# Dylan-H-Wang/skin-sm3

Measured on AMD Instinct MI355X. Metric: SM3 pretrain images/sec (paired 224x224), higher is better.
Workload: dtype bf16

## Files before the change

### include/sm3_hip.h

```cpp
#ifndef SM3_HIP_H
#define SM3_HIP_H

#include <stdint.h>

#ifdef __cplusplus
extern "C" {
#endif

#define SM3_F32 0
#define SM3_BF16 1
#define SM3_F16 2

#define SM3_EINVAL (-1)
#define SM3_EALIGN (-2)
#define SM3_EDTYPE (-3)

#define SM3_MAX_TAPS 9

int sm3_abi_version(void);

typedef struct sm3_conv_desc {
    int32_t dtype;
    int32_t N, Hi, Wi, Ci;
    int32_t Ho, Wo, Co;
// ... 54 lines not shown
int sm3_conv_wgrad_slabs(const sm3_conv_desc* d, const void* x, const void* dy, float* slabs, int slab_capacity, int views,
                         int* slabs_used, void* stream);
int sm3_slab_reduce(const float* slabs, int nslabs, int64_t n, float* out, int accumulate, void* stream);
int sm3_conv_wgrad_det(const sm3_conv_desc* d, const void* x, const void* dy, float* dw, float* slabs, int slab_capacity,
                       void* stream);

#define SM3_BN_REDUCE_GROUPS 64
int sm3_bn_reduce_groups(int rows);
int sm3_bn_stats_reduce(const float* partials, int rows, int C, double* sums, double* workspace, int views,
                        void* stream);
int sm3_bn_finalize(const double* sums, int groups , int views,
                    double count , int C, const float* gamma, const float* beta,
                    float eps, float momentum, float* running_mean, float* running_var,
                    int64_t* num_batches_tracked , float* scale, float* shift, float* save_mean,
                    float* save_invstd , void* stream);
int sm3_bn_eval_scale_shift(const float* gamma, const float* beta, const float* running_mean,
                            const float* running_var, float eps, int C, float* scale, float* shift,
                            void* stream);
int sm3_bn_act(int dtype, const void* x, const float* scale, const float* shift, const void* residual,
               int relu, int out_f32, void* y, uint8_t* relu_mask, int64_t rows, int C, int views, void* stream);
int sm3_bn_act_colsum_rows(int64_t rows, int C, int dtype);
int sm3_bn_act_colsum(int dtype, const void* x, const float* scale, const float* shift, const void* residual, int relu,
                      void* y, uint8_t* relu_mask, float* colsum_partials, int64_t rows, int C, int views, void* stream);
int sm3_subsample_colsum_rows(int64_t rows, int C, int dtype);
int sm3_subsample_colsum(int dtype, const void* x, void* y, float* colsum_partials, int N, int H, int W, int C, int stride,
                         int views, void* stream);
int sm3_bn_add_bn_act(int dtype, const void* x, const float* scale, const float* shift, const void* x2,
                      const float* scale2, const float* shift2, int relu, void* y, uint8_t* relu_mask,
                      int64_t rows, int C, int views, void* stream);
int sm3_bn_bwd_partial_rows(int64_t rows, int C);
int sm3_bn_bwd_reduce(int dtype, const void* dy, const void* y, const uint8_t* relu_mask, const void* x,
                      const float* mean, const float* invstd, void* dz, int64_t rows, int C,
                      float* partials , int views, void* stream);
int sm3_bn_bwd_apply(int dtype, const void* dz, const void* x, const float* mean, const float* invstd,
                     const float* gamma, const double* global_sums, double count,
                     const double* local_sums, float* dgamma, float* dbeta, void* dx, int64_t rows,
                     int C, int views, void* stream);

typedef struct sm3_bn_apply_side {
    const void* x;
    const float* mean;
    const float* invstd;
    const float* gamma;
    const double* global_sums;
    const double* local_sums;
    float* dgamma;
// ... 246 lines not shown
```

### skin-sm3_amd/csrc/bn.hip

```cpp
#include "common.h"
#include <cstdlib>

namespace {

struct RowWalk {
    int tbx, tby;
    int gx, gy;
};
static RowWalk make_walk(int64_t rows, int cvecs, int max_gy, int views = 1) {
    RowWalk w;
    if (cvecs >= 256) {
        w.tbx = 256;
    } else {
        w.tbx = cvecs;
    }
    w.tby = 256 / w.tbx;
    if (w.tby < 1) w.tby = 1;
    w.gx = (cvecs + w.tbx - 1) / w.tbx;
    int64_t gy = (rows + (int64_t)w.tby * 8 - 1) / ((int64_t)w.tby * 8);
    static const int grid_cap = getenv("SM3_BN_GRID_CAP") ? atoi(getenv("SM3_BN_GRID_CAP")) : 768;
    const int64_t cap = grid_cap / (w.gx * views) > 0 ? grid_cap / (w.gx * views) : 1;
    if (gy > cap) gy = cap;
    if (gy > max_gy) gy = max_gy;
    if (gy < 1) gy = 1;
// ... 269 lines not shown
#pragma unroll
                for (int e = 0; e < E; ++e) cs[e] += q[e];
            }
        }
        for (; r < rows; r += rstep) {
            const uint4 xu = ldg16<false>(x + src_row(r) * C + (int64_t)cv * E);
            if (y) stg16<true>(y + (r_lo + r) * C + (int64_t)cv * E, xu);
            float q[E];
            unpack16<T>(xu, q);
#pragma unroll
            for (int e = 0; e < E; ++e) cs[e] += q[e];
        }
    }
    if constexpr (E <= 8) {
#pragma unroll
        for (int e = 0; e < E; ++e) scol[threadIdx.x * E + e] = cs[e];
    }
    __syncthreads();
    if (active && ty == 0) {
        for (int j = 1; j < tby; ++j)
#pragma unroll
            for (int e = 0; e < E; ++e) cs[e] += scol[(j * tbx + tx) * E + e];
        float* o = colsum + ((int64_t)blockIdx.z * gridDim.y + blockIdx.y) * C + (int64_t)cv * E;
#pragma unroll
        for (int e = 0; e < E; ++e) o[e] = cs[e];
    }
}

template <typename T, int U, bool NT>
__global__ __launch_bounds__(256) void bn_bwd_reduce_kernel(const T* __restrict__ dy, const T* __restrict__ y,
                                                            const uint8_t* __restrict__ mask,
                                                            const T* __restrict__ x, const float* __restrict__ mean,
                                                            const float* __restrict__ invstd, T* __restrict__ dz,
                                                            int64_t rows, int C, float* __restrict__ partials,
                                                            int tbx, int tby) {
    constexpr int E = ElemTraits<T>::kPer16B;
    __shared__ float sred[256 * 2 * 8];
    const int tx = threadIdx.x % tbx, ty = threadIdx.x / tbx;
    const int cv = blockIdx.x * tbx + tx;
    const bool active = (cv * E < C) && (ty < tby);
    {
        const int64_t vo = (int64_t)blockIdx.z * rows * C;
        dy += vo;
        if (x) {
            x += vo;
            mean += (int64_t)blockIdx.z * C;
// ... 392 lines not shown
    if (!SM3_DTYPE_OK(dtype)) return SM3_EDTYPE;
    const int E = dtype == SM3_F32 ? 4 : 8;
    if (C % E) return SM3_EALIGN;
    const int Hs = (H - 1) / stride + 1, Ws = (W - 1) / stride + 1;
    const int64_t rows = (int64_t)(N / views) * Hs * Ws;
    if ((int64_t)N * Hs * Ws > 0x7fffffffL) return SM3_EINVAL;
    const RowWalk w = make_walk(rows, C / E, 8192, views < 2 ? 2 : views);
    dim3 grid(w.gx, w.gy, views), block(256);
    const FastDiv dhw = make_fastdiv((uint32_t)(Hs * Ws)), dw = make_fastdiv((uint32_t)Ws);
    hipStream_t st = (hipStream_t)stream;
    if (dtype == SM3_F32)
        hipLaunchKernelGGL((subsample_colsum_kernel<float, 4>), grid, block, 0, st, (const float*)x, (float*)y, colsum_partials, rows,
                           C, Hs, Ws, H, W, stride, dhw, dw, w.tbx, w.tby);
    else if (dtype == SM3_BF16)
        hipLaunchKernelGGL((subsample_colsum_kernel<bf16_t, 4>), grid, block, 0, st, (const bf16_t*)x, (bf16_t*)y, colsum_partials,
                           rows, C, Hs, Ws, H, W, stride, dhw, dw, w.tbx, w.tby);
    else
        hipLaunchKernelGGL((subsample_colsum_kernel<f16_t, 4>), grid, block, 0, st, (const f16_t*)x, (f16_t*)y, colsum_partials,
                           rows, C, Hs, Ws, H, W, stride, dhw, dw, w.tbx, w.tby);
    SM3_CHECK_LAUNCH();
    return 0;
}

extern "C" int sm3_bn_add_bn_act(int dtype, const void* x, const float* scale, const float* shift, const void* x2,
                                 const float* scale2, const float* shift2, int relu, void* y, uint8_t* relu_mask,
                                 int64_t rows, int C, int views, void* stream) {
    if (!x2 || !scale2 || !shift2) return SM3_EINVAL;
    return bn_act_impl(dtype, x, scale, shift, x2, scale2, shift2, relu, 0, y, relu_mask, rows, C, views, stream);
}

static int bwd_gy(int64_t rows) {
    int64_t gy = (rows + 63) / 64;
    if (gy > 1024) gy = 1024;
    if (gy < 1) gy = 1;
    return (int)gy;
}

extern "C" int sm3_bn_bwd_partial_rows(int64_t rows, int C) {
    (void)C;
    return rows > 0 ? bwd_gy(rows) : SM3_EINVAL;
}

extern "C" int sm3_bn_bwd_reduce(int dtype, const void* dy, const void* y, const uint8_t* relu_mask, const void* x,
                                 const float* mean, const float* invstd, void* dz, int64_t rows, int C,
                                 float* partials, int views, void* stream) {
    if (!dy || (x && (!mean || !invstd)) || !partials || rows <= 0 || C <= 0 || views < 1) return SM3_EINVAL;
// ... 74 lines not shown
```

### skin-sm3_amd/sm3hip/_lib.py

```python
import ctypes as C
import os

_HERE = os.path.dirname(os.path.abspath(__file__))
LIB_PATH = os.environ.get("SM3_LIBRARY") or os.path.join(_HERE, "libsm3hip.so")

SM3_F32, SM3_BF16, SM3_F16 = 0, 1, 2
MAX_TAPS = 9


class ConvDesc(C.Structure):
    _fields_ = [
        ("dtype", C.c_int32),
        ("N", C.c_int32), ("Hi", C.c_int32), ("Wi", C.c_int32), ("Ci", C.c_int32),
        ("Ho", C.c_int32), ("Wo", C.c_int32), ("Co", C.c_int32),
        ("sy", C.c_int32), ("sx", C.c_int32),
        ("ntaps", C.c_int32),
        ("dy", C.c_int32 * MAX_TAPS), ("dx", C.c_int32 * MAX_TAPS), ("wtap", C.c_int32 * MAX_TAPS),
        ("w_row_stride", C.c_int32),
        ("Hout", C.c_int32), ("Wout", C.c_int32),
        ("osy", C.c_int32), ("osx", C.c_int32), ("ooy", C.c_int32), ("oox", C.c_int32),
    ]


class BnBwdFuse(C.Structure):
# ... 27 lines not shown
    "sm3_conv_gather_gemm": [_DESC, _P, _P, _P, _P, _P, _P],
    "sm3_conv_dgrad_bnfuse": [_DESC, _P, _P, _P, _P, _P, _P],
    "sm3_conv_dgrad_seg_bnfuse": [_DESC, _P, _P, _P, _P, _P, _P, _P],
    "sm3_conv_gather_gemm_seg": [_DESC, _P, _P, _P, _P, _P, _P],
    "sm3_conv_seg_act": [_DESC, _P, _P, _P, _I, _P, _P, _P],
    "sm3_linbn_fold": [_P, _I, _I, _I, _P, _P],
    "sm3_p2p_mailbox_bytes": [],
    "sm3_p2p_max_elems": [],
    "sm3_p2p_max_world": [],
    "sm3_p2p_layout": [_I, _I, _I, _P, _P, _P, _P],
    "sm3_p2p_alloc": [_P, _P, _P],
    "sm3_p2p_open": [_P, _P],
    "sm3_p2p_close": [_P],
    "sm3_p2p_free": [_P],
    "sm3_p2p_allreduce_f64": [_P, _I, _P, _I, _I, C.c_uint64, _P, _D, _P],
    "sm3_linbn_scale_banks": [_I, _P, _I, _P, _P, _P, _P, _I, _P, _P, _P, _P, _I, _I, _P],
    "sm3_subsample_colsum_rows": [_L, _I, _I],
    "sm3_subsample_colsum": [_I, _P, _P, _P, _I, _I, _I, _I, _I, _I, _P],
    "sm3_conv_wgrad_cat": [_DESC, _P, _P, _P, _P, _I, _P, _I, _L, _L, _P],
    "sm3_bn_act_colsum_rows": [_L, _I, _I],
    "sm3_conv_wgrad_slabs": [_DESC, _P, _P, _P, _I, _I, _P, _P],
    "sm3_linbn_moments": [_P, _I, _L, _P, _P, _I, _P, _I, _I, _P],
    "sm3_bn_act_colsum": [_I, _P, _P, _P, _P, _I, _P, _P, _P, _L, _I, _I, _P],
    "sm3_conv_bn_act_fused": [_DESC, _P, _P, _P, _P, _P, _I, _P, _P, _I, _P],
    "sm3_linbn_fwd_stats": [_I, _P, _P, _P, _P, _P, _P, _I, _I, _I, _P],
    "sm3_linbn_stats": [_I, _P, _P, _P, _P, _P, _P, _I, _P, _P, _P, _D, _P, _I, _I, _I, _P],
    "sm3_linbn_coef": [_P, _D, _P, _P, _P, _P, _I, _I, _P],
    "sm3_linbn_banks": [_I, _P, _P, _P, _P, _P, _I, _I, _I, _P],
    "sm3_linbn_post": [_I, _P, _P, _P, _P, _P, _P, _P, _P, _P, _I, _I, _I, _P],
    "sm3_linbn_banks_post": [_I, _P, _P, _P, _P, _P, _P, _P, _P, _P, _P, _I, _I, _I, _P],
    "sm3_conv_bn_act_eval": [_DESC, _P, _P, _P, _P, _P, _I, _P, _P],
    "sm3_conv_bn_eval": [_DESC, _P, _P, _P, _P, _P, _P, _F, _P, _I, _P, _P],
    "sm3_conv_wgrad": [_DESC, _P, _P, _P, _P],
    "sm3_conv_wgrad_det": [_DESC, _P, _P, _P, _P, _I, _P],
    "sm3_slab_reduce": [_P, _I, _L, _P, _I, _P],
    "sm3_bn_stats_reduce": [_P, _I, _I, _P, _P, _I, _P],
    "sm3_bn_reduce_groups": [_I],
    "sm3_bn_finalize": [_P, _I, _I, _D, _I, _P, _P, _F, _F, _P, _P, _P, _P, _P, _P, _P, _P],
    "sm3_bn_eval_scale_shift": [_P, _P, _P, _P, _F, _I, _P, _P, _P],
    "sm3_bn_act": [_I, _P, _P, _P, _P, _I, _I, _P, _P, _L, _I, _I, _P],
    "sm3_bn_add_bn_act": [_I, _P, _P, _P, _P, _P, _P, _I, _P, _P, _L, _I, _I, _P],
    "sm3_bn_bwd_apply2": [_I, _P, _D, _P, _P, _L, _I, _I, _P],
    "sm3_bn_relu_maxpool_fwd": [_I, _P, _P, _P, _P, _P, _I, _I, _I, _I, _I, _P],
    "sm3_maxpool_bn_bwd_partial_rows": [_I, _I, _I, _I],
    "sm3_maxpool_bn_bwd": [_I, _P, _P, _P, _P, _P, _P, _P, _P, _P, _I, _I, _I, _I, _I, _P],
    "sm3_bn_bwd_partial_rows": [_L, _I],
# ... 131 lines not shown
```

### skin-sm3_amd/sm3hip/engine.py

```python
import os
from collections import OrderedDict
from contextlib import contextmanager

import torch

from . import ops
from ._lib import SM3_BF16, SM3_F16
from .plan import (TWO_PASS, BlockRec, EncoderCtx, ParamStore, ProjectorPlan, Rec, block_form, enc_mod_out_dim, enc_plan,
                   stage_of)
from .plan import EncoderPlan

BN_EPS = 1e-5
BN_MOMENTUM = 0.1


_LANE_POOL = {}


def lane_stream_pool(device, n):
    idx = device.index if device.index is not None else torch.cuda.current_device()
    pool = _LANE_POOL.setdefault(idx, [])
    if len(pool) >= n:
        return pool[:n]
    if os.environ.get("SM3_STREAM_CALIBRATE", "1") == "0" or not hasattr(torch.cuda, "_sleep"):
        pool.extend(torch.cuda.Stream(device=device) for _ in range(n - len(pool)))
        return pool[:n]
    import time
    main = torch.cuda.current_stream(device)
    cyc = 1_000_000

    def spin(a, b):
        torch.cuda.synchronize(device)
        t0 = time.perf_counter()
        with torch.cuda.stream(a):
            torch.cuda._sleep(cyc)
# ... 62 lines not shown
        self._allocated = False
        self._lane = "main"
        self._V = 1
        self._data_only = False
        self._no_stat_update = False
        self.weights_dirty = True
        self._wprep_cache, self._wprep_key, self._hash_tracks_banks = {}, None, False
        self._lane_prep = {}
        self._lin_descs = {}
        self.last_feats = None
        self._faith_saved_bytes = {}
        self.pair_views = os.environ.get("SM3_PAIR_VIEWS", "1") != "0"
        self.two_streams = True
        self._streams, self._streams_dev = None, None
        self.linbn = self.dtype in (SM3_BF16, SM3_F16) and os.environ.get("SM3_LINBN", "1") != "0"
        self.linbn_fwd = os.environ.get("SM3_LINBN_FWD", "1") != "0"
        self.linbn_ds = os.environ.get("SM3_LINBN_DS", "1") != "0"
        self.linbn_join = os.environ.get("SM3_LINBN_JOIN", "1") != "0"
        self.linbn_merge = os.environ.get("SM3_LINBN_MERGE", "1") != "0"
        self.lane_cross = os.environ.get("SM3_LANE_CROSS", "1") != "0"
        if self.cross is not None and self.cross[0] is self.cross[1]:
            self.lane_cross = False
        self.det_wgrad = os.environ.get("SM3_WGRAD_DET", "1") != "0"
        self.stem16 = self.dtype in (SM3_BF16, SM3_F16) and os.environ.get("SM3_STEM16", "1") != "0"

    def _all_conv_units(self):
        seen = set()
        plans = [p for pair in self.branches.values() for p in pair if p is not None]
        plans += list(self.cross or ())
        if self.meta is not None:
            plans.append(self.meta)
        for plan in plans:
            for cu in plan.conv_units():
                if id(cu) not in seen:
                    seen.add(id(cu))
                    yield cu

    def prepare(self, device):
        if self.store is None or self.store.flat_p.device != device:
            self.store = ParamStore(self.module, device)
            self._allocated = False
        else:
            self.store.rebind_if_needed()
        if not self._allocated:
            for cu in self._all_conv_units():
                cu.alloc(self.dtype, device)
# ... 131 lines not shown
            rm, rv = self.buffers[bu.name + ".running_mean"], self.buffers[bu.name + ".running_var"]
            nbt = self.buffers[bu.name + ".num_batches_tracked"]
        ops.bn_finalize(sums, count, bu.C, gamma, beta, BN_EPS, BN_MOMENTUM, rm, rv, nbt, scale, shift, mean, invstd,
                        groups=groups, views=V)

    @contextmanager
    def _views(self, V):
        self._V = V
        try:
            yield
        finally:
            self._V = 1

    @contextmanager
    def _params_backward(self, params):
        prev = self._data_only
        self._data_only = prev or not params
        try:
            yield
        finally:
            self._data_only = prev

    def conv_bn(self, cu, bu, x, N, H, W, relu, residual=None, train=True, save=False, out_f32=False, y_out=None,
                apply=True, scale_shift=None, res_affine=None, pending=None, colsum=None):
        dev = x.t.device if isinstance(x, ops.StemImage) else x.device
        direct = cu.stem
        if direct:
            d = None
            Ho, Wo = (H - 1) // 2 + 1, (W - 1) // 2 + 1
        else:
            d = cu.fwd_desc(self.dtype, N, H, W)
            Ho, Wo = d.Ho, d.Wo
        rows = N * Ho * Wo
        C = cu.Co
        V = self._V if train else 1
        rows_v = rows // V
        xo = torch.empty(rows, C, dtype=self.tdt, device=dev)
        scale, shift = scale_shift if scale_shift is not None else (self._work("scale", 2 * 2048),
                                                                    self._work("shift", 2 * 2048))
        mean = invstd = None

        def convolve(partials):
            if direct:
                (ops.stem_conv_fwd16 if isinstance(x, ops.StemImage) else ops.stem_conv_fwd)(self.dtype, x, cu.w_fwd, xo, partials)
            elif cu.groups > 1:
                ops.gconv_fwd(self.dtype, x, cu.w_fwd, xo, partials, N, H, W, C, cu.groups, cu.stride)
            else:
# ... 45 lines not shown
                if y_out is None:
                    y_out = xo
                ops.conv_bn_eval(d, x, cu.w_fwd, gamma, beta, rm, rv, BN_EPS, residual, relu, y_out)
                return y_out, Ho, Wo, None
            convolve(None)
            ops.bn_eval_scale_shift(gamma, beta, rm, rv, BN_EPS, C, scale, shift)
            if save:
                mean, invstd = rm.clone(), torch.rsqrt(rv + BN_EPS)
        mask = None
        if not apply:
            y_out = None
        else:
            if y_out is None:
                y_out = torch.empty(rows, C, dtype=torch.float32 if out_f32 else self.tdt, device=dev)
            if save and relu:
                mask = torch.empty(rows * C // (16 // ops._sz(self.dtype)), dtype=torch.uint8, device=dev)
            cs = None
            if res_affine is not None:
                ops.bn_add_bn_act(self.dtype, xo, scale, shift, residual, res_affine[0], res_affine[1], relu, y_out,
                                  rows_v, C, mask=mask, views=V)
            else:
                if colsum is not None and save and train and not out_f32:
                    cs = colsum
                ops.bn_act(self.dtype, xo, scale, shift, residual, relu, y_out, rows_v, C, out_f32=out_f32, mask=mask,
                           views=V, colsum=cs)
        r = None
        if save:
            r = Rec(cu, bu, N, H, W, Ho, Wo, x_in=x, xo=xo, mean=mean, invstd=invstd, y=y_out, relu=relu, mask=mask, V=V,
                    frozen_stats=not train, colsum=cs if apply else None)
        return (y_out if apply else xo), Ho, Wo, r

    def _phase1(self, r, dy, fused_rows):
        if fused_rows is not None:
            return fused_rows, self._ws[(self._lane, "fz_partials")]
        C, V = r.cu.Co, r.V
        rows = r.N * r.Ho * r.Wo // V
        prow = ops.bn_bwd_partial_rows(rows, C)
        bpart = self._work("partials", V * prow * 2 * C)
        ops.bn_bwd_reduce(self.dtype, dy, None, r.xo, r.mean, r.invstd, dy if r.relu else None, rows, C, bpart,
                          mask=r.mask if r.relu else None, views=V)
        return prow, bpart

    def bn_backward(self, r, dy, keep_dz, fused_rows=None):
        C = r.cu.Co
        V = r.V
        rows = r.xo.shape[0] // V
        prow, bpart = self._phase1(r, dy, fused_rows)
        lsums, gsums, count = self._bn_backward_sums(r, bpart, prow)
# ... 32 lines not shown
        ops.bn_stats_reduce(dpart, prow_d, C, lsums[n:], views=V)
        gsums, count = lsums, rows
        if r3.frozen_stats:
            gsums = self._work("zsums2", 2 * 2 * 2 * 2048, torch.float64)
            gsums.zero_()
        elif self.stat_sync is not None:
            gsums = self._work("gsums2", 2 * 2 * 2 * 2048, torch.float64)
            gsums[: 2 * n].copy_(lsums[: 2 * n])
            self.stat_sync(gsums[: 2 * n])
            count = rows * self.world_size
        dx3 = torch.empty_like(r3.xo)

        def side(r, g, l, dx):
            dgamma, dbeta = self._bn_affine(r.bu, grad=True)
            return dict(x=r.xo, mean=r.mean, invstd=r.invstd, gamma=self._bn_affine(r.bu)[0], gsums=g, lsums=l,
                        dgamma=dgamma, dbeta=dbeta, dx=dx)
        ops.bn_bwd_apply2(self.dtype, dy, count, side(r3, gsums[:n], lsums[:n], dx3),
                          side(rd, gsums[n: 2 * n], lsums[n: 2 * n], dy), rows, C, views=V)
        return dx3, dy

    def _slab_buf(self, n, V):
        cap = max(1, min(ops.SLAB_CAP, (1 << 24) // n))
        return self._work("linbn_slabs", V * cap * n), cap

    def _lin_conv_desc(self, dtype, N, H, W, Ci, Co):
        cache = self._lin_descs
        key = ("conv", dtype, N, H, W, Ci, Co)
        if key not in cache:
            cache[key] = ops.fwd_desc(dtype, N, H, W, Ci, Co, 1, 1, 0)
        return cache[key]

    def conv3_bn3_fused(self, cu, bu, r2, y2, idn, N, H, W):
        dev = y2.device
        C, p, V = cu.Co, cu.Ci, self._V
        d = cu.fwd_desc(self.dtype, N, H, W)
        rows = N * d.Ho * d.Wo
        rows_v = rows // V
        if V > 1 and rows_v % 128:
            raise ValueError("two views in one batch need a multiple of 128 rows per view")
        Tm = torch.empty(V * C * p, dtype=torch.float32, device=dev)
        groups = p // 32
        ws = self._work("linbn_fws", V * groups * 2 * C, torch.float64)
        ops.linbn_fwd_stats(self.dtype, r2.gram, cu.w_dgrad, cu.w_fwd, r2.colsum, Tm, ws, C, p, V)
        count = rows_v
        if self.stat_sync is not None:
            gs = self._work("linbn_fold", 2 * V * 2 * C, torch.float64)
# ... 41 lines not shown
        for bu, wsl, groups, tag in units:
            scale, shift = self._work("scale" + tag, 2 * 2048), self._work("shift" + tag, 2 * 2048)
            mean = torch.empty(V * C, dtype=torch.float32, device=dev)
            invstd = torch.empty(V * C, dtype=torch.float32, device=dev)
            self._bn_finalize(bu, wsl, count, scale, shift, mean, invstd, groups, V)
            out.append((scale, shift, mean, invstd))
        (sc3, sh3, mean3, inv3), (scd, shd, meand, invd) = out
        w3s = self._work("linbn_w3s", V * C * p, self.tdt)
        wds = self._work("linbn_wds", V * C * Cin, self.tdt)
        bias = self._work("linbn_fbias", V * C)
        ops.linbn_scale_banks(self.dtype, c3.w_fwd, sc3, sh3, w3s, cd.w_fwd, scd, shd, wds, bias, C, V)
        y3 = torch.empty(M, C, dtype=self.tdt, device=dev)
        mask = torch.empty(M * C // (16 // ops._sz(self.dtype)), dtype=torch.uint8, device=dev)
        ops.conv_seg_act(self._lin_conv_desc(self.dtype, N, h2, w2, p, C), y2, w3s, in_s, wds, bias, y3, mask, True,
                         views=V, w_view_stride=C * p, w1_view_stride=C * Cin)
        rd = Rec(cd, bd, N, h, w, h2, w2, x_in=cur, mean=meand, invstd=invd, V=V, linbn=True, in_s=in_s, gram=Gd, colsum=sd,
                 Tm=Tmd)
        r3 = Rec(c3, b3, N, h2, w2, h2, w2, x_in=y2, mean=mean3, invstd=inv3, y=y3, relu=True, mask=mask, V=V, linbn=True,
                 Tm=Tm3)
        return y3, h2, w2, rd, r3

    def _strided_input_moments(self, cd, x, N, h, w, hs, ws, V, keep):
        Cin, M = cd.Ci, N * hs * ws
        crow = ops.subsample_colsum_rows(self.dtype, M // V, Cin)
        csd = self._work("linbn_cs", V * crow * Cin)
        in_s = x if cd.stride == 1 else torch.empty(M, Cin, dtype=self.tdt, device=x.device)
        ops.subsample_colsum(self.dtype, x, None if cd.stride == 1 else in_s, csd, N, h, w, Cin, cd.stride, V)
        slabs, cap = self._slab_buf(Cin * Cin, V)
        ns = ops.conv_wgrad_slabs(self._lin_conv_desc(self.dtype, N, hs, ws, Cin, Cin), in_s, in_s, slabs, views=V, cap=cap)
        if keep:
            Gd = torch.empty(V * Cin * Cin, dtype=torch.float32, device=x.device)
            sd = torch.empty(V * Cin, dtype=torch.float64, device=x.device)
        else:
            Gd = self._work("linbn_Gd", V * Cin * Cin)
            sd = self._work("linbn_sd", V * Cin, torch.float64)
        ops.linbn_moments(slabs, ns, Cin * Cin, Gd, views=V, colsum=csd, colsum_rows=crow, s_out=sd, p=Cin)
        return in_s, Gd, sd

    def _lin_unit_products(self, tag, cu, N, Hs, Ws, y_in, dz, V):
        C, p = cu.Co, cu.Ci
        slabs, cap = self._slab_buf(C * p, V)
        ns = ops.conv_wgrad_slabs(self._lin_conv_desc(self.dtype, N, Hs, Ws, p, C), y_in, dz, slabs, views=V, cap=cap)
        P = self._work("linbn_P" + tag, V * C * p)
        ops.linbn_moments(slabs, ns, C * p, P, views=V)
        return P

    def _lin_unit_finish(self, tag, cu, P, G, Tm, s, coef, V):
        C, p = cu.Co, cu.Ci
        wa = self._work("linbn_wa" + tag, V * p * C, self.tdt)
        cconst = self._work("linbn_const" + tag, V * p)
        Hn = self._work("linbn_H" + tag, V * p * p, self.tdt)
        if self.linbn_merge:
# ... 206 lines not shown

    def _identity_branch(self, blk, cur, N, h, w, train, save):
        if "cd" not in blk:
            return cur, None, None, None
        if not (train or save):
            return self.conv_bn(blk["cd"], blk["bd"], cur, N, h, w, False, None, train)[0], None, None, None
        ra = (self._work("scale_d", 2 * 2048), self._work("shift_d", 2 * 2048))
        pend = [] if (train and self.stat_sync is not None) else None
        idn, _, _, rd = self.conv_bn(blk["cd"], blk["bd"], cur, N, h, w, False, None, train, save, apply=False,
                                     scale_shift=ra, pending=pend)
        return idn, ra, pend, rd

    def _basic_forward(self, blk, form, cur, N, h, w, train, save):
        y1, h1, w1, r1 = self.conv_bn(blk["c1"], blk["b1"], cur, N, h, w, True, None, train, save)
        idn, ra, pend, rd = self._identity_branch(blk, cur, N, h, w, train, save)
        y2, h2, w2, r2 = self.conv_bn(blk["c2"], blk["b2"], y1, N, h1, w1, True, idn, train, save, res_affine=ra,
                                      pending=pend)
        return y2, h2, w2, (BlockRec(form, r1, r2, rd=rd) if save else None)

    def _bottleneck_forward(self, blk, form, cur, N, h, w, train, save):
        V = self._V
        y1, h1, w1, r1 = self.conv_bn(blk["c1"], blk["b1"], cur, N, h, w, True, None, train, save)
        pp = blk["c3"].Ci
        cs = crow = None
        if form.lin:
            d2 = blk["c2"].fwd_desc(self.dtype, N, h1, w1)
            crow = ops.bn_act_colsum_rows(self.dtype, N * d2.Ho * d2.Wo // V, pp)
            cs = self._work("linbn_cs", V * crow * pp)
        y2, h2, w2, r2 = self.conv_bn(blk["c2"], blk["b2"], y1, N, h1, w1, True, None, train, save, colsum=cs)
        if form.lin:
            slabs, cap = self._slab_buf(pp * pp, V)
            ns = ops.conv_wgrad_slabs(self._lin_conv_desc(self.dtype, N, h2, w2, pp, pp), y2, y2, slabs, views=V, cap=cap)
            r2.gram = torch.empty(V * pp * pp, dtype=torch.float32, device=y2.device)
            r2.colsum = torch.empty(V * pp, dtype=torch.float64, device=y2.device)
            ops.linbn_moments(slabs, ns, pp * pp, r2.gram, views=V, colsum=cs, colsum_rows=crow, s_out=r2.colsum, p=pp)
        if form.join_fused:
            y3, h3, w3, rd, r3 = self.join_fused(blk, r2, y2, cur, N, h, w, h2, w2)
        else:
            idn, ra, pend, rd = self._identity_branch(blk, cur, N, h, w, train, save)
            if form.conv3_fused:
                y3, h3, w3, r3 = self.conv3_bn3_fused(blk["c3"], blk["b3"], r2, y2, idn, N, h2, w2)
            else:
                y3, h3, w3, r3 = self.conv_bn(blk["c3"], blk["b3"], y2, N, h2, w2, True, idn, train, save, res_affine=ra,
                                              pending=pend)
                if form.lin:
                    r3.linbn = True
        return y3, h3, w3, (BlockRec(form, r1, r2, r3, rd) if save else None)

    def encoder_backward(self, ctx, dfeat, last_view=True, taps=None, dx_out=None, params=True, stop_at=None):
        with self._params_backward(params):
            return self._encoder_backward(ctx, dfeat, last_view, taps, dx_out, stop_at)

    def _stop_block(self, ctx, stop_at):
        names = [stage_of(b) for b in ctx.plan.blocks]
        if stop_at not in names or names[-1] == stop_at:
# ... 326 lines not shown
```

### skin-sm3_amd/sm3hip/ops.py

```python
import ctypes as C

import torch

from . import _lib
from ._lib import ConvDesc, SM3_BF16, SM3_F16, SM3_F32, check

TORCH_DTYPE = {SM3_F32: torch.float32, SM3_BF16: torch.bfloat16, SM3_F16: torch.float16}
K_CHUNK = {SM3_F32: 32, SM3_BF16: 64, SM3_F16: 64}


_PROFILER = None


def set_profiler(p):
    global _PROFILER
    _PROFILER = p


class _prof:
    __slots__ = ("tag", "flops", "nbytes", "start")

    def __init__(self, tag, flops=0.0, nbytes=0.0):
        self.tag, self.flops, self.nbytes, self.start = tag, flops, nbytes, None

# ... 836 lines not shown
    if x.numel() != n or y.numel() != n or (residual is not None and residual.numel() != n):
        raise ValueError("bn_act: size mismatch")
    if scale.numel() < views * Cn or shift.numel() < views * Cn:
        raise ValueError("bn_act: scale/shift too small")
    _chk(mask, torch.uint8, "mask")
    if mask is not None and mask.numel() != n // (16 // _sz(dtype)):
        raise ValueError("bn_act: mask size mismatch")
    tag = "bn_act"
    if _PROFILER is not None and getattr(_PROFILER, "detail", False):
        tag += f"|rows{views * rows}_C{Cn}_res{int(residual is not None)}"
    _chk(colsum, torch.float32, "colsum")
    if colsum is not None and (out_f32 or colsum.numel() < views * bn_act_colsum_rows(dtype, rows, Cn) * Cn):
        raise ValueError("bn_act: colsum needs the storage dtype and [views][colsum_rows][C] floats")
    with _prof(tag, 0.0, _sz(dtype) * n * (2 if residual is None else 3)):
        if colsum is not None:
            check(_lib.load().sm3_bn_act_colsum(dtype, _ptr(x), _ptr(scale), _ptr(shift), _ptr(residual), int(relu),
                                                _ptr(y), _ptr(mask), _ptr(colsum), rows, Cn, views, _stream()),
                  "sm3_bn_act_colsum")
        else:
            check(_lib.load().sm3_bn_act(dtype, _ptr(x), _ptr(scale), _ptr(shift), _ptr(residual), int(relu),
                                         int(out_f32), _ptr(y), _ptr(mask), rows, Cn, views, _stream()), "sm3_bn_act")


def bn_add_bn_act(dtype, x, scale, shift, x2, scale2, shift2, relu, y, rows, Cn, mask=None, views=1):
    tdt = TORCH_DTYPE[dtype]
    for t in (x, x2, y):
        _chk(t, tdt)
    for t in (scale, shift, scale2, shift2):
        _chk(t, torch.float32)
        if t.numel() < views * Cn:
            raise ValueError("bn_add_bn_act: scale/shift too small")
    n = views * rows * Cn
    if x.numel() != n or x2.numel() != n or y.numel() != n:
        raise ValueError("bn_add_bn_act: size mismatch")
    _chk(mask, torch.uint8, "mask")
    if mask is not None and mask.numel() != n // (16 // _sz(dtype)):
        raise ValueError("bn_add_bn_act: mask size mismatch")
    tag = "bn_act"
    if _PROFILER is not None and getattr(_PROFILER, "detail", False):
        tag += f"|rows{views * rows}_C{Cn}_res2"
    with _prof(tag, 0.0, _sz(dtype) * n * 3):
        check(_lib.load().sm3_bn_add_bn_act(dtype, _ptr(x), _ptr(scale), _ptr(shift), _ptr(x2), _ptr(scale2),
                                            _ptr(shift2), int(relu), _ptr(y), _ptr(mask), rows, Cn, views, _stream()),
              "sm3_bn_add_bn_act")


# ... 1004 lines not shown
```

Before: 4641.

## Fuse BN-apply with Gram and column-sum moments in one MFMA kernel

Adds a kernel that applies BN scale/shift and ReLU, writes the output and mask, and also accumulates the per-slab Gram matrix (with MFMA on a double-buffered LDS tile) and column sums in the same pass. The engine uses it for the lin-BN conv2 output and for stride-1 input moments when C=64 and the tensor is large enough. This replaces a separate bn_act_colsum or subsample pass followed by a wgrad-based Gram launch, removing a second full read of the activation. The cost is a heavier kernel that may run at lower occupancy and produces more partial slabs to reduce.

Result: no change. 4655, median of 6 (+0.3%).

```diff
diff --git a/include/sm3_hip.h b/include/sm3_hip.h
--- a/include/sm3_hip.h
+++ b/include/sm3_hip.h
@@ -100,6 +100,9 @@
 int sm3_bn_act_colsum_rows(int64_t rows, int C, int dtype);
 int sm3_bn_act_colsum(int dtype, const void* x, const float* scale, const float* shift, const void* residual, int relu,
                       void* y, uint8_t* relu_mask, float* colsum_partials, int64_t rows, int C, int views, void* stream);
+int sm3_bn_act_gram_rows(int64_t rows, int C, int dtype);
+int sm3_bn_act_gram(int dtype, const void* x, const float* scale, const float* shift, int relu, void* y, uint8_t* relu_mask,
+                    float* slabs, float* colsum_partials, int64_t rows, int C, int views, void* stream);
 int sm3_subsample_colsum_rows(int64_t rows, int C, int dtype);
 int sm3_subsample_colsum(int dtype, const void* x, void* y, float* colsum_partials, int N, int H, int W, int C, int stride,
                          int views, void* stream);
diff --git a/scratch/bn_act_gram_ab.py b/scratch/bn_act_gram_ab.py
--- /dev/null
+++ b/scratch/bn_act_gram_ab.py
@@ -0,0 +1,109 @@
+import sys
+import torch
+
+sys.path.insert(0, "skin-sm3_amd")
+from sm3hip import ops
+
+D = torch.device("cuda:0")
+NSET, ITERS, ALTS = 3, 6, 5
+
+
+def timed(fn):
+    torch.cuda.synchronize()
+    a, b = torch.cuda.Event(enable_timing=True), torch.cuda.Event(enable_timing=True)
+    a.record()
+    for i in range(ITERS):
+        fn(i % NSET)
+    b.record()
+    torch.cuda.synchronize()
+    return a.elapsed_time(b) * 1e3 / ITERS
+
+
+def shape(C, rows, V, dt, out):
+    code = ops.dtype_code(dt)
+    n = V * rows * C
+    xs = [torch.randn(n // 64, 64, device=D).to(dt).reshape(V * rows, C) for _ in range(NSET)]
+    ys = [torch.empty_like(x) for x in xs]
+    ms = [torch.empty(n // 8, dtype=torch.uint8, device=D) for _ in range(NSET)]
+    scale, shift = torch.rand(V * C, device=D) + 0.5, torch.randn(V * C, device=D) * 0.3
+    crow = ops.bn_act_colsum_rows(code, rows, C)
+    cs0 = torch.empty(V * crow * C, device=D)
+    cap = max(1, min(ops.SLAB_CAP, (1 << 24) // (C * C)))
+    slabs0 = torch.empty(V * cap * C * C, device=D)
+    R = ops.bn_act_gram_rows(code, rows, C)
+    cs1 = torch.empty(V * R * C, device=D)
+    slabs1 = torch.empty(V * R * C * C, device=D)
+    desc = ops.fwd_desc(code, V, rows, 1, C, C, 1, 1, 0)
+    G = torch.empty(V * C * C, device=D)
+    s = torch.empty(V * C, dtype=torch.float64, device=D)
+    ns = [0]
+
+    def plain(i):
+        ops.bn_act(code, xs[i], scale, shift, None, True, ys[i], rows, C, mask=ms[i], views=V)
+
+    def colsum(i):
+        ops.bn_act(code, xs[i], scale, shift, None, True, ys[i], rows, C, mask=ms[i], views=V, colsum=cs0)
+
+    def gram(i):
+        ns[0] = ops.conv_wgrad_slabs(desc, ys[i], ys[i], slabs0, views=V, cap=cap)
+
+    def two(i):
+        colsum(i)
+        gram(i)
+        ops.linbn_moments(slabs0, ns[0], C * C, G, views=V, colsum=cs0, colsum_rows=crow, s_out=s, p=C)
+
+    def fused(i):
+        ops.bn_act_gram(code, xs[i], scale, shift, True, ys[i], rows, C, slabs1, cs1, mask=ms[i], views=V)
+        ops.linbn_moments(slabs1, R, C * C, G, views=V, colsum=cs1, colsum_rows=R, s_out=s, p=C)
+
+    def fused_alone(i):
+        ops.bn_act_gram(code, xs[i], scale, shift, True, ys[i], rows, C, slabs1, cs1, mask=ms[i], views=V)
+
+    def sub(i):
+        ops.subsample_colsum(code, xs[i], None, cs0, V, rows, 1, C, 1, V)
+
+    def two_m(i):
+        sub(i)
+        ns[0] = ops.conv_wgrad_slabs(desc, xs[i], xs[i], slabs0, views=V, cap=cap)
+        ops.linbn_moments(slabs0, ns[0], C * C, G, views=V, colsum=cs0, colsum_rows=crow, s_out=s, p=C)
+
+    def fused_m(i):
+        ops.bn_act_gram(code, xs[i], None, None, False, None, rows, C, slabs1, cs1, views=V)
+        ops.linbn_moments(slabs1, R, C * C, G, views=V, colsum=cs1, colsum_rows=R, s_out=s, p=C)
+
+    fns = [("bn_act", plain), ("bn_act_colsum", colsum), ("gram_wgrad", gram), ("two_launches+moments", two),
+           ("fused+moments", fused), ("fused_alone", fused_alone), ("subsample+gram+moments", two_m), ("moments_only+moments", fused_m)]
+    for _, f in fns:
+        for i in range(NSET):
+            f(i)
+    mb = 2 * n * 2 / 1e6
+    out.write(f"\n== C={C} rows/view={rows} views={V} {str(dt).split('.')[-1]}: y = {mb / 2:.0f} MB, slabs per view: wgrad {ns[0]}, "
+              f"fused {R}\n")
+    out.write("alt " + " ".join(f"{k:>24s}" for k, _ in fns) + "   (us per call)\n")
+    res = {k: [] for k, _ in fns}
+    for a in range(ALTS):
+        row = []
+        for k, f in fns:
+            t = timed(f)
+            res[k].append(t)
+            row.append(t)
+        out.write(f"{a:3d} " + " ".join(f"{t:24.1f}" for t in row) + "\n")
+    t2, tf, tp = res["two_launches+moments"], res["fused+moments"], res["bn_act"]
+    ta = res["fused_alone"]
+    out.write(f"apply: fused faster in every alternation: {all(f < t for f, t in zip(tf, t2))}; "
+              f"fused launch alone / bn_act alone (medians): {sorted(ta)[ALTS // 2] / sorted(tp)[ALTS // 2]:.3f}; "
+              f"plain pass {mb / sorted(tp)[ALTS // 2] :.2f} TB/s\n")
+    t2, tf = res["subsample+gram+moments"], res["moments_only+moments"]
+    out.write(f"moments only: fused faster in every alternation: {all(f < t for f, t in zip(tf, t2))}\n")
+    out.flush()
+
+
+if __name__ == "__main__":
+    path = sys.argv[1] if len(sys.argv) > 1 else "profiles/bn_act_gram_per_shape.txt"
+    with open(path, "w") as out:
+        out.write("sm3_bn_act_gram per shape, single lane, interleaved in one process; 3 buffer sets rotate (cold HBM reads)\n")
+        for C, rows, V, dt in [(64, 802816, 2, torch.bfloat16), (128, 200704, 2, torch.bfloat16),
+                               (64, 802816, 2, torch.float16), (128, 200704, 2, torch.float16),
+                               (64, 401408, 2, torch.bfloat16), (128, 100352, 2, torch.bfloat16),
+                               (64, 100352, 2, torch.bfloat16), (128, 25088, 2, torch.bfloat16)]:
+            shape(C, rows, V, dt, out)
diff --git a/skin-sm3_amd/csrc/bn.hip b/skin-sm3_amd/csrc/bn.hip
--- a/skin-sm3_amd/csrc/bn.hip
+++ b/skin-sm3_amd/csrc/bn.hip
@@ -315,6 +315,193 @@
 #pragma unroll
             for (int e = 0; e < E; ++e) cs[e] += scol[(j * tbx + tx) * E + e];
         float* o = colsum + ((int64_t)blockIdx.z * gridDim.y + blockIdx.y) * C + (int64_t)cv * E;
+#pragma unroll
+        for (int e = 0; e < E; ++e) o[e] = cs[e];
+    }
+}
+
+template <int ROW_BYTES>
+__device__ __forceinline__ uint32_t gram_swz(int row) {
+    if constexpr (ROW_BYTES >= 256) return (uint32_t)(row & 3) << 6;
+    else return (uint32_t)((row >> 1) & 1) << 6;
+}
+template <typename T>
+__device__ __forceinline__ void gram_mma(const uint4& a, const uint4& b, f32x16& c);
+template <>
+__device__ __forceinline__ void gram_mma<bf16_t>(const uint4& a, const uint4& b, f32x16& c) {
+    c = __builtin_amdgcn_mfma_f32_32x32x16_bf16(__builtin_bit_cast(bf16x8, a), __builtin_bit_cast(bf16x8, b), c, 0, 0, 0);
+}
+template <>
+__device__ __forceinline__ void gram_mma<f16_t>(const uint4& a, const uint4& b, f32x16& c) {
+    c = __builtin_amdgcn_mfma_f32_32x32x16_f16(__builtin_bit_cast(f16x8, a), __builtin_bit_cast(f16x8, b), c, 0, 0, 0);
+}
+
+template <typename T, int P, int NW, int U, bool MOMENTS, bool NT>
+__global__ __launch_bounds__(NW * 64, (P == 64 ? 3 : 1) * (NW / 4)) void bn_act_gram_kernel(const T* __restrict__ x, const float* __restrict__ scale,
+                                                          const float* __restrict__ shift, int relu, T* __restrict__ y,
+                                                          uint8_t* __restrict__ mask, int64_t rows,
+                                                          float* __restrict__ slabs, float* __restrict__ colsum) {
+    constexpr int E = 8, TBX = P / E, TBY = NW * 64 / TBX, SW = TBY * U;
+    constexpr int RB = P * 2, TILE = SW * RB;
+    constexpr int WNW = NW / 2, WTM = P / 2, WTN = P / WNW;
+    constexpr int TM = WTM / 32, TN = WTN / 32;
+    constexpr int NCH = P == 64 ? 2 : 1;
+    static_assert(sizeof(T) == 2 && (P == 64 || P == 128) && TN >= 1 && SW % 16 == 0, "16-bit types, 64 or 128 channels");
+    __shared__ __attribute__((aligned(16))) char tile[2 * TILE];
+    __shared__ float scol[NW * 64 * E];
+    const int tx = threadIdx.x % TBX, ty = threadIdx.x / TBX;
+    const int lane = threadIdx.x & 63, wave = threadIdx.x >> 6, wm = wave / WNW, wn = wave % WNW;
+    {
+        const int64_t vo = (int64_t)blockIdx.z * rows * P;
+        x += vo;
+        if constexpr (!MOMENTS) {
+            y += vo;
+            if (mask) mask += (int64_t)blockIdx.z * rows * TBX;
+            scale += (int64_t)blockIdx.z * P;
+            shift += (int64_t)blockIdx.z * P;
+        }
+    }
+    float sc[E], sh[E], cs[E];
+#pragma unroll
+    for (int e = 0; e < E; ++e) {
+        sc[e] = MOMENTS ? 1.f : scale[tx * E + e];
+        sh[e] = MOMENTS ? 0.f : shift[tx * E + e];
+        cs[e] = 0.f;
+    }
+    auto finish = [&](int64_t r, const uint4& xu) {
+        if (r >= rows) return make_uint4(0, 0, 0, 0);
+        uint4 pk = xu;
+        if constexpr (!MOMENTS) {
+            float v[E];
+            unpack16<T>(xu, v);
+#pragma unroll
+            for (int e = 0; e < E; ++e) v[e] = v[e] * sc[e] + sh[e];
+            if (relu) {
+                if (mask) {
+                    constexpr float thr = ElemTraits<T>::kReluBit;
+                    unsigned m = 0;
+#pragma unroll
+                    for (int e = 0; e < E; ++e) m |= (v[e] > thr ? 1u : 0u) << e;
+                    mask[r * TBX + tx] = (uint8_t)m;
+                }
+#pragma unroll
+                for (int e = 0; e < E; ++e) v[e] = relu_f32(v[e]);
+            }
+            pk = pack16<T>(v);
+            stg16<NT>(y + r * P + tx * E, pk);
+        }
+        float q[E];
+        unpack16<T>(pk, q);
+#pragma unroll
+        for (int e = 0; e < E; ++e) cs[e] += q[e];
+        return pk;
+    };
+    const int64_t rstep = (int64_t)gridDim.y * TBY;
+    const int64_t rb = (int64_t)blockIdx.y * TBY, r0 = rb + ty;
+    const int64_t nk = rb < rows ? (rows - rb + rstep - 1) / rstep : 0;
+    const int64_t nsweeps = (nk + U - 1) / U;
+    uint4 xu[U];
+    auto issue = [&](int64_t s) {
+#pragma unroll
+        for (int u = 0; u < U; ++u) {
+            const int64_t r = r0 + (s * U + u) * rstep;
+            xu[u] = r < rows ? ldg16<NT>(x + r * P + tx * E) : make_uint4(0, 0, 0, 0);
+        }
+    };
+
+    f32x16 acc[TM][TN];
+#pragma unroll
+    for (int i = 0; i < TM; ++i)
+#pragma unroll
+        for (int j = 0; j < TN; ++j)
+#pragma unroll
+            for (int r = 0; r < 16; ++r) acc[i][j][r] = 0.f;
+    uint32_t ra_off[TM], rb_off[TN];
+    {
+        const int g = lane >> 4, ii = lane & 15, q = ii >> 2, pq = ii & 3, h = g >> 1;
+        const int colsel = 16 * (g & 1) + 4 * pq;
+        const int krow0 = 8 * h + q;
+#pragma unroll
+        for (int i = 0; i < TM; ++i)
+            ra_off[i] = (uint32_t)krow0 * RB + (((uint32_t)(wm * WTM + i * 32 + colsel) * 2u) ^ gram_swz<RB>(q));
+#pragma unroll
+        for (int j = 0; j < TN; ++j)
+            rb_off[j] = (uint32_t)krow0 * RB + (((uint32_t)(wn * WTN + j * 32 + colsel) * 2u) ^ gram_swz<RB>(q));
+    }
+
+    if (nsweeps > 0) issue(0);
+    for (int64_t s = 0; s < nsweeps; ++s) {
+        char* const tb = tile + (int)(s & 1) * TILE;
+#pragma unroll
+        for (int u = 0; u < U; ++u) {
+            const uint4 pk = finish(r0 + (s * U + u) * rstep, xu[u]);
+            const int t = u * TBY + ty;
+            *reinterpret_cast<uint4*>(tb + t * RB + (((uint32_t)tx * 16u) ^ gram_swz<RB>(t))) = pk;
+        }
+        if (s + 1 < nsweeps) issue(s + 1);
+        __syncthreads();
+        f32x16 part[NCH][TM][TN];
+#pragma unroll
+        for (int c = 0; c < NCH; ++c)
+#pragma unroll
+            for (int i = 0; i < TM; ++i)
+#pragma unroll
+                for (int j = 0; j < TN; ++j)
+#pragma unroll
+                    for (int r = 0; r < 16; ++r) part[c][i][j][r] = 0.f;
+#pragma unroll
+        for (int ks = 0; ks < SW / 16; ++ks) {
+            uint4 fa[TM], fb[TN];
+#pragma unroll
+            for (int i = 0; i < TM; ++i) {
+                const char* a0 = tb + ra_off[i] + ks * 16 * RB;
+                const s16x4 lo = __builtin_amdgcn_ds_read_tr16_b64_v4i16((__attribute__((address_space(3))) s16x4*)(a0));
+                const s16x4 hi = __builtin_amdgcn_ds_read_tr16_b64_v4i16((__attribute__((address_space(3))) s16x4*)(a0 + 4 * RB));
+                const uint2 l2 = __builtin_bit_cast(uint2, lo), h2 = __builtin_bit_cast(uint2, hi);
+                fa[i] = make_uint4(l2.x, l2.y, h2.x, h2.y);
+            }
+#pragma unroll
+            for (int i = 0; i < TN; ++i) {
+                const char* b0 = tb + rb_off[i] + ks * 16 * RB;
+                const s16x4 lob = __builtin_amdgcn_ds_read_tr16_b64_v4i16((__attribute__((address_space(3))) s16x4*)(b0));
+                const s16x4 hib = __builtin_amdgcn_ds_read_tr16_b64_v4i16((__attribute__((address_space(3))) s16x4*)(b0 + 4 * RB));
+                const uint2 lb = __builtin_bit_cast(uint2, lob), hb = __builtin_bit_cast(uint2, hib);
+                fb[i] = make_uint4(lb.x, lb.y, hb.x, hb.y);
+            }
+#pragma unroll
+            for (int i = 0; i < TM; ++i)
+#pragma unroll
+                for (int j = 0; j < TN; ++j) gram_mma<T>(fa[i], fb[j], part[ks % NCH][i][j]);
+        }
+#pragma unroll
+        for (int i = 0; i < TM; ++i)
+#pragma unroll
+            for (int j = 0; j < TN; ++j) {
+                if constexpr (NCH == 2) acc[i][j] += part[0][i][j] + part[1][i][j];
+                else acc[i][j] += part[0][i][j];
+            }
+    }
+
+    float* const so = slabs + ((int64_t)blockIdx.z * gridDim.y + blockIdx.y) * (P * P);
+    const int frow = lane & 31, fh = lane >> 5;
+#pragma unroll
+    for (int i = 0; i < TM; ++i)
+#pragma unroll
+        for (int j = 0; j < TN; ++j)
+#pragma unroll
+            for (int r = 0; r < 16; ++r) {
+                const int c0 = wm * WTM + i * 32 + (r & 3) + 8 * (r >> 2) + 4 * fh;
+                const int c1 = wn * WTN + j * 32 + frow;
+                so[c0 * P + c1] = acc[i][j][r];
+            }
+#pragma unroll
+    for (int e = 0; e < E; ++e) scol[threadIdx.x * E + e] = cs[e];
+    __syncthreads();
+    if (ty == 0) {
+        for (int j = 1; j < TBY; ++j)
+#pragma unroll
+            for (int e = 0; e < E; ++e) cs[e] += scol[(j * TBX + tx) * E + e];
+        float* o = colsum + ((int64_t)blockIdx.z * gridDim.y + blockIdx.y) * P + tx * E;
 #pragma unroll
         for (int e = 0; e < E; ++e) o[e] = cs[e];
     }
@@ -753,6 +940,52 @@
     return 0;
 }
 
+extern "C" int sm3_bn_act_gram_rows(int64_t rows, int C, int dtype) {
+    if (rows <= 0 || (C != 64 && C != 128) || (dtype != SM3_BF16 && dtype != SM3_F16)) return 0;
+    int64_t n = rows / (16 * (int64_t)C);
+    const int64_t cap = C == 64 ? 384 : 128;
+    if (n > cap) n = cap;
+    return n < 1 ? 1 : (int)n;
+}
+
+extern "C" int sm3_bn_act_gram(int dtype, const void* x, const float* scale, const float* shift, int relu, void* y,
+                               uint8_t* relu_mask, float* slabs, float* colsum_partials, int64_t rows, int C, int views,
+                               void* stream) {
+    if (!x || !slabs || !colsum_partials || rows <= 0 || C <= 0 || views < 1) return SM3_EINVAL;
+    const bool moments = !y;
+    if (moments ? (scale || shift || relu_mask) : (!scale || !shift)) return SM3_EINVAL;
+    if (!SM3_DTYPE_OK(dtype)) return SM3_EDTYPE;
+    if (dtype == SM3_F32) return SM3_EDTYPE;
+    if (C != 64 && C != 128) return SM3_EALIGN;
+    dim3 grid(1, sm3_bn_act_gram_rows(rows, C, dtype), views);
+    hipStream_t st = (hipStream_t)stream;
+#define SM3_GRAM_K(T, P, NW, U, M, NT)                                                                                  \
+    hipLaunchKernelGGL((bn_act_gram_kernel<T, P, NW, U, M, NT>), grid, dim3(NW * 64), 0, st, (const T*)x, scale, shift, \
+                       relu, (T*)y, relu_mask, rows, slabs, colsum_partials)
+#define SM3_GRAM_C(T, P, NW, U, NT)                        \
+    do {                                                   \
+        if (moments) SM3_GRAM_K(T, P, NW, U, true, false); \
+        else SM3_GRAM_K(T, P, NW, U, false, NT);           \
+    } while (0)
+#define SM3_GRAM_T(T, NT)                              \
+    do {                                               \
+        if (C == 64) SM3_GRAM_C(T, 64, 4, 4, NT);      \
+        else SM3_GRAM_C(T, 128, 8, 4, NT);             \
+    } while (0)
+    if (bn_nt()) {
+        if (dtype == SM3_BF16) SM3_GRAM_T(bf16_t, true);
+        else SM3_GRAM_T(f16_t, true);
+    } else {
+        if (dtype == SM3_BF16) SM3_GRAM_T(bf16_t, false);
+        else SM3_GRAM_T(f16_t, false);
+    }
+#undef SM3_GRAM_T
+#undef SM3_GRAM_C
+#undef SM3_GRAM_K
+    SM3_CHECK_LAUNCH();
+    return 0;
+}
+
 extern "C" int sm3_bn_add_bn_act(int dtype, const void* x, const float* scale, const float* shift, const void* x2,
                                  const float* scale2, const float* shift2, int relu, void* y, uint8_t* relu_mask,
                                  int64_t rows, int C, int views, void* stream) {
diff --git a/skin-sm3_amd/sm3hip/_lib.py b/skin-sm3_amd/sm3hip/_lib.py
--- a/skin-sm3_amd/sm3hip/_lib.py
+++ b/skin-sm3_amd/sm3hip/_lib.py
@@ -73,6 +73,8 @@
     "sm3_conv_wgrad_slabs": [_DESC, _P, _P, _P, _I, _I, _P, _P],
     "sm3_linbn_moments": [_P, _I, _L, _P, _P, _I, _P, _I, _I, _P],
     "sm3_bn_act_colsum": [_I, _P, _P, _P, _P, _I, _P, _P, _P, _L, _I, _I, _P],
+    "sm3_bn_act_gram_rows": [_L, _I, _I],
+    "sm3_bn_act_gram": [_I, _P, _P, _P, _I, _P, _P, _P, _P, _L, _I, _I, _P],
     "sm3_conv_bn_act_fused": [_DESC, _P, _P, _P, _P, _P, _I, _P, _P, _I, _P],
     "sm3_linbn_fwd_stats": [_I, _P, _P, _P, _P, _P, _P, _I, _I, _I, _P],
     "sm3_linbn_stats": [_I, _P, _P, _P, _P, _P, _P, _I, _P, _P, _P, _D, _P, _I, _I, _I, _P],
diff --git a/skin-sm3_amd/sm3hip/engine.py b/skin-sm3_amd/sm3hip/engine.py
--- a/skin-sm3_amd/sm3hip/engine.py
+++ b/skin-sm3_amd/sm3hip/engine.py
@@ -11,6 +11,8 @@
 from .plan import EncoderPlan
 
 BN_EPS = 1e-5
+BN_GRAM_MIN_BYTES = 12 << 20
+BN_GRAM_WIDTHS = "64"
 BN_MOMENTUM = 0.1
 
 
@@ -119,6 +121,9 @@
         if self.cross is not None and self.cross[0] is self.cross[1]:
             self.lane_cross = False
         self.det_wgrad = os.environ.get("SM3_WGRAD_DET", "1") != "0"
+        self.bn_gram = os.environ.get("SM3_BN_GRAM", "1") != "0"
+        self.bn_gram_min_bytes = int(os.environ.get("SM3_BN_GRAM_MIN_BYTES", str(BN_GRAM_MIN_BYTES)))
+        self.bn_gram_widths = tuple(int(c) for c in os.environ.get("SM3_BN_GRAM_C", BN_GRAM_WIDTHS).split(",") if c)
         self.stem16 = self.dtype in (SM3_BF16, SM3_F16) and os.environ.get("SM3_STEM16", "1") != "0"
 
     def _all_conv_units(self):
@@ -296,7 +301,7 @@
             self._data_only = prev
 
     def conv_bn(self, cu, bu, x, N, H, W, relu, residual=None, train=True, save=False, out_f32=False, y_out=None,
-                apply=True, scale_shift=None, res_affine=None, pending=None, colsum=None):
+                apply=True, scale_shift=None, res_affine=None, pending=None, colsum=None, gram=None):
         dev = x.t.device if isinstance(x, ops.StemImage) else x.device
         direct = cu.stem
         if direct:
@@ -388,8 +393,11 @@
             else:
                 if colsum is not None and save and train and not out_f32:
                     cs = colsum
-                ops.bn_act(self.dtype, xo, scale, shift, residual, relu, y_out, rows_v, C, out_f32=out_f32, mask=mask,
-                           views=V, colsum=cs)
+                if cs is not None and gram is not None and residual is None:
+                    ops.bn_act_gram(self.dtype, xo, scale, shift, relu, y_out, rows_v, C, gram, cs, mask=mask, views=V)
+                else:
+                    ops.bn_act(self.dtype, xo, scale, shift, residual, relu, y_out, rows_v, C, out_f32=out_f32, mask=mask,
+                               views=V, colsum=cs)
         r = None
         if save:
             r = Rec(cu, bu, N, H, W, Ho, Wo, x_in=x, xo=xo, mean=mean, invstd=invstd, y=y_out, relu=relu, mask=mask, V=V,
@@ -468,6 +476,12 @@
     def _slab_buf(self, n, V):
         cap = max(1, min(ops.SLAB_CAP, (1 << 24) // n))
         return self._work("linbn_slabs", V * cap * n), cap
+
+    def _bn_gram_rows(self, rows_v, C):
+        if (not self.bn_gram or self.dtype not in (SM3_BF16, SM3_F16) or C not in self.bn_gram_widths
+                or rows_v * C * ops._sz(self.dtype) < self.bn_gram_min_bytes):
+            return 0
+        return ops.bn_act_gram_rows(self.dtype, rows_v, C)
 
     def _lin_conv_desc(self, dtype, N, H, W, Ci, Co):
         cache = self._lin_descs
@@ -555,12 +569,19 @@
 
     def _strided_input_moments(self, cd, x, N, h, w, hs, ws, V, keep):
         Cin, M = cd.Ci, N * hs * ws
-        crow = ops.subsample_colsum_rows(self.dtype, M // V, Cin)
-        csd = self._work("linbn_cs", V * crow * Cin)
-        in_s = x if cd.stride == 1 else torch.empty(M, Cin, dtype=self.tdt, device=x.device)
-        ops.subsample_colsum(self.dtype, x, None if cd.stride == 1 else in_s, csd, N, h, w, Cin, cd.stride, V)
-        slabs, cap = self._slab_buf(Cin * Cin, V)
-        ns = ops.conv_wgrad_slabs(self._lin_conv_desc(self.dtype, N, hs, ws, Cin, Cin), in_s, in_s, slabs, views=V, cap=cap)
+        ns = self._bn_gram_rows(M // V, Cin) if cd.stride == 1 else 0
+        if ns > 0:
+            in_s, crow = x, ns
+            csd = self._work("linbn_cs", V * crow * Cin)
+            slabs = self._work("linbn_slabs", V * ns * Cin * Cin)
+            ops.bn_act_gram(self.dtype, x, None, None, False, None, M // V, Cin, slabs, csd, views=V)
+        else:
+            crow = ops.subsample_colsum_rows(self.dtype, M // V, Cin)
+            csd = self._work("linbn_cs", V * crow * Cin)
+            in_s = x if cd.stride == 1 else torch.empty(M, Cin, dtype=self.tdt, device=x.device)
+            ops.subsample_colsum(self.dtype, x, None if cd.stride == 1 else in_s, csd, N, h, w, Cin, cd.stride, V)
+            slabs, cap = self._slab_buf(Cin * Cin, V)
+            ns = ops.conv_wgrad_slabs(self._lin_conv_desc(self.dtype, N, hs, ws, Cin, Cin), in_s, in_s, slabs, views=V, cap=cap)
         if keep:
             Gd = torch.empty(V * Cin * Cin, dtype=torch.float32, device=x.device)
             sd = torch.empty(V * Cin, dtype=torch.float64, device=x.device)
@@ -813,15 +834,23 @@
         V = self._V
         y1, h1, w1, r1 = self.conv_bn(blk["c1"], blk["b1"], cur, N, h, w, True, None, train, save)
         pp = blk["c3"].Ci
-        cs = crow = None
+        cs = crow = slabs = None
+        ns = 0
         if form.lin:
             d2 = blk["c2"].fwd_desc(self.dtype, N, h1, w1)
-            crow = ops.bn_act_colsum_rows(self.dtype, N * d2.Ho * d2.Wo // V, pp)
+            rows_v = N * d2.Ho * d2.Wo // V
+            ns = self._bn_gram_rows(rows_v, pp) if (save and train) else 0
+            if ns > 0:
+                crow = ns
+                slabs = self._work("linbn_slabs", V * ns * pp * pp)
+            else:
+                crow = ops.bn_act_colsum_rows(self.dtype, rows_v, pp)
             cs = self._work("linbn_cs", V * crow * pp)
-        y2, h2, w2, r2 = self.conv_bn(blk["c2"], blk["b2"], y1, N, h1, w1, True, None, train, save, colsum=cs)
+        y2, h2, w2, r2 = self.conv_bn(blk["c2"], blk["b2"], y1, N, h1, w1, True, None, train, save, colsum=cs, gram=slabs)
         if form.lin:
-            slabs, cap = self._slab_buf(pp * pp, V)
-            ns = ops.conv_wgrad_slabs(self._lin_conv_desc(self.dtype, N, h2, w2, pp, pp), y2, y2, slabs, views=V, cap=cap)
+            if ns == 0:
+                slabs, cap = self._slab_buf(pp * pp, V)
+                ns = ops.conv_wgrad_slabs(self._lin_conv_desc(self.dtype, N, h2, w2, pp, pp), y2, y2, slabs, views=V, cap=cap)
             r2.gram = torch.empty(V * pp * pp, dtype=torch.float32, device=y2.device)
             r2.colsum = torch.empty(V * pp, dtype=torch.float64, device=y2.device)
             ops.linbn_moments(slabs, ns, pp * pp, r2.gram, views=V, colsum=cs, colsum_rows=crow, s_out=r2.colsum, p=pp)
diff --git a/skin-sm3_amd/sm3hip/ops.py b/skin-sm3_amd/sm3hip/ops.py
--- a/skin-sm3_amd/sm3hip/ops.py
+++ b/skin-sm3_amd/sm3hip/ops.py
@@ -882,6 +882,39 @@
                                          int(out_f32), _ptr(y), _ptr(mask), rows, Cn, views, _stream()), "sm3_bn_act")
 
 
+def bn_act_gram_rows(dtype, rows, Cn):
+    return _lib.load().sm3_bn_act_gram_rows(rows, Cn, dtype)
+
+
+def bn_act_gram(dtype, x, scale, shift, relu, y, rows, Cn, slabs, colsum, mask=None, views=1):
+    tdt = TORCH_DTYPE[dtype]
+    _chk(x, tdt, "x"); _chk(y, tdt, "y"); _chk(scale, torch.float32); _chk(shift, torch.float32)
+    _chk(slabs, torch.float32, "slabs"); _chk(colsum, torch.float32, "colsum")
+    n = views * rows * Cn
+    if x.numel() != n or (y is not None and y.numel() != n):
+        raise ValueError("bn_act_gram: size mismatch")
+    if y is None:
+        if scale is not None or shift is not None or mask is not None:
+            raise ValueError("bn_act_gram: moments only takes neither scale / shift nor a mask")
+    elif scale is None or shift is None or scale.numel() < views * Cn or shift.numel() < views * Cn:
+        raise ValueError("bn_act_gram: scale/shift too small")
+    _chk(mask, torch.uint8, "mask")
+    if mask is not None and mask.numel() != n // (16 // _sz(dtype)):
+        raise ValueError("bn_act_gram: mask size mismatch")
+    R = bn_act_gram_rows(dtype, rows, Cn)
+    if R < 1:
+        raise ValueError("bn_act_gram: 64 or 128 channels of a 16-bit type")
+    if slabs is None or colsum is None or slabs.numel() < views * R * Cn * Cn or colsum.numel() < views * R * Cn:
+        raise ValueError("bn_act_gram: slabs / colsum need [views][bn_act_gram_rows][C][C] / [C] floats")
+    tag = "bn_act_gram"
+    if _PROFILER is not None and getattr(_PROFILER, "detail", False):
+        tag += f"|rows{views * rows}_C{Cn}" + ("_moments" if y is None else "")
+    with _prof(tag, 2.0 * views * rows * Cn * Cn, _sz(dtype) * n * (1 if y is None else 2) + 4 * views * R * Cn * Cn):
+        check(_lib.load().sm3_bn_act_gram(dtype, _ptr(x), _ptr(scale), _ptr(shift), int(relu), _ptr(y), _ptr(mask),
+                                          _ptr(slabs), _ptr(colsum), rows, Cn, views, _stream()), "sm3_bn_act_gram")
+    return R
+
+
 def bn_add_bn_act(dtype, x, scale, shift, x2, scale2, shift2, relu, y, rows, Cn, mask=None, views=1):
     tdt = TORCH_DTYPE[dtype]
     for t in (x, x2, y):
```
